# ChengeLi/LongTerm360FoV

Measured on AMD Instinct MI355X. Metric: sequences/sec (batch=1024, T_in=30->T_out=30, h=256), higher is better.
Workload: dtype f32; 1 GPU; configs[1]: target-only seq2seq inference (encoder + autoregressive decoder), H=256, batch=1024 per GPU, T_in=30->T_out=30, F_enc=90, F_dec=6, fp32, act=sigmoid, impl=auto; global_batch=1024, parallelism=replicas x1 (no collective)

## Files before the change

### longterm360fov_amd/csrc/lstm_cluster.hip

```cpp
#include <stdlib.h>

#include <atomic>
#include <mutex>

#include "fov_common.h"
#include "xch_common.h"

namespace fov {

constexpr int BT = 16;
constexpr int XR = 6;
constexpr int KPAD = 2;
constexpr int NXBUF = 3;
constexpr int CL_MAX_F = 96;
constexpr int CL_MAX_O = 8;

constexpr int MODE_LAYER = 0;
constexpr int MODE_DECODE = 1;
constexpr int MODE_LAYER_ZX = 2;

typedef unsigned u32x2 __attribute__((ext_vector_type(2)));
typedef unsigned u32x4g __attribute__((ext_vector_type(4)));
typedef float f32x2 __attribute__((ext_vector_type(2)));
template <bool V> struct BoolC { static constexpr bool value = V; };

__device__ __forceinline__ unsigned long long ld_granule(const unsigned long long* p) {
    return __hip_atomic_load(p, __ATOMIC_RELAXED, __HIP_MEMORY_SCOPE_AGENT);
}
__device__ __forceinline__ void st_granule(unsigned long long* p, unsigned long long v) {
    __hip_atomic_store(p, v, __ATOMIC_RELAXED, __HIP_MEMORY_SCOPE_AGENT);
}
__device__ __forceinline__ void st_granule_l2(unsigned long long* p, unsigned long long v) {
    __hip_atomic_store(p, v, __ATOMIC_RELAXED, __HIP_MEMORY_SCOPE_WORKGROUP);
}
__device__ __forceinline__ unsigned xcc_id() {
    unsigned x;
    asm volatile("s_getreg_b32 %0, hwreg(HW_REG_XCC_ID, 0, 4)" : "=s"(x));
    return x;
}

__host__ __device__ constexpr int round16(int v) { return (v + 15) & ~15; }

#ifdef FOV_STAMPS
constexpr int STAMP_SLOTS = 12;
constexpr int STAMP_STEPS = 64;
__device__ unsigned long long g_stamps[2][STAMP_STEPS][STAMP_SLOTS];
#define FOV_STAMP(slot)                                                                         \
    do {                                                                                        \
        __builtin_amdgcn_sched_barrier(0);                                                      \
        if (stamp_on && t < STAMP_STEPS) {                                                      \
            unsigned long long t_;                                                              \
            asm volatile("s_memtime %0\n\ts_waitcnt lgkmcnt(0)" : "=s"(t_)::"memory");          \
            g_stamps[MODE & 1][t][slot] = t_;                                                       \
        }                                                                                       \
        __builtin_amdgcn_sched_barrier(0);                                                      \
    } while (0)
#define FOV_PSTAMP(slot)                                                                        \
    do {                                                                                        \
        __builtin_amdgcn_sched_barrier(0);                                                      \
        if (blockIdx.x == 5 && threadIdx.x == 0) g_stamps[MODE & 1][STAMP_STEPS - 1][slot] = __builtin_amdgcn_s_memtime(); \
        __builtin_amdgcn_sched_barrier(0);                                                      \
    } while (0)
#else
#define FOV_STAMP(slot) do { } while (0)
#define FOV_PSTAMP(slot) do { } while (0)
#endif

struct ClusterLds {
    int ldx, ldh;
    int off_k, off_h, off_x, off_w, off_bd, off_flag, total_floats;
};
__host__ __device__ inline ClusterLds cluster_lds(int H, int F, bool decode) {
    ClusterLds L;
    const int fp = round16(F);
    L.ldx = fp + 4;
    L.ldh = H + 4;
    L.off_k = 0;
    L.off_h = L.off_k + fp * 256 + 4 * KPAD * 256;
    L.off_x = L.off_h + BT * L.ldh;
    L.off_w = L.off_x + NXBUF * BT * L.ldx;
    L.off_bd = L.off_w + (decode ? 2 * 4 * 128 : 0);
    L.off_flag = L.off_bd + 8;
    L.total_floats = L.off_flag + 8 + 64;
    return L;
}

constexpr int MF_MID = 0, MF_FIRST = 1, MF_LAST = 2;
#define FOV_MFMA_STR(pre, post) pre "v_mfma_f32_16x16x4_f32 %0, %1, %2, %0" post
template <bool W_AGPR>
__device__ __forceinline__ void mfma_f32(f32x4& acc, float a, float w, int pos) {
    if constexpr (W_AGPR) {
        if (pos == MF_MID) asm volatile(FOV_MFMA_STR("", "") : "+v"(acc) : "v"(a), "a"(w));
        else if (pos == MF_FIRST) asm volatile(FOV_MFMA_STR("s_nop 1\n\t", "") : "+v"(acc) : "v"(a), "a"(w));
        else if (pos == MF_LAST) asm volatile(FOV_MFMA_STR("", "\n\ts_nop 7\n\ts_nop 3") : "+v"(acc) : "v"(a), "a"(w));
        else asm volatile(FOV_MFMA_STR("s_nop 1\n\t", "\n\ts_nop 7\n\ts_nop 3") : "+v"(acc) : "v"(a), "a"(w));
    } else {
        if (pos == MF_MID) asm volatile(FOV_MFMA_STR("", "") : "+v"(acc) : "v"(a), "v"(w));
        else if (pos == MF_FIRST) asm volatile(FOV_MFMA_STR("s_nop 1\n\t", "") : "+v"(acc) : "v"(a), "v"(w));
        else if (pos == MF_LAST) asm volatile(FOV_MFMA_STR("", "\n\ts_nop 7\n\ts_nop 3") : "+v"(acc) : "v"(a), "v"(w));
        else asm volatile(FOV_MFMA_STR("s_nop 1\n\t", "\n\ts_nop 7\n\ts_nop 3") : "+v"(acc) : "v"(a), "v"(w));
    }
}
#define FOV_MFMA_C_STR(pre) pre "v_mfma_f32_16x16x4_f32 %0, %1, %2, %3"
template <bool W_AGPR>
__device__ __forceinline__ void mfma_f32_c(f32x4& acc, float a, float w, const f32x4& c, bool a_fresh) {
    if constexpr (W_AGPR) {
        if (a_fresh) asm volatile(FOV_MFMA_C_STR("s_nop 1\n\t") : "=&v"(acc) : "v"(a), "a"(w), "v"(c));
        else asm volatile(FOV_MFMA_C_STR("") : "=&v"(acc) : "v"(a), "a"(w), "v"(c));
    } else {
        if (a_fresh) asm volatile(FOV_MFMA_C_STR("s_nop 1\n\t") : "=&v"(acc) : "v"(a), "v"(w), "v"(c));
        else asm volatile(FOV_MFMA_C_STR("") : "=&v"(acc) : "v"(a), "v"(w), "v"(c));
    }
}
__host__ __device__ constexpr int mf_pos(bool first_run, bool last_run, bool is_first, bool is_last) {
    return ((first_run && is_first) ? MF_FIRST : 0) | ((last_run && is_last) ? MF_LAST : 0);
}

template <int H, bool DEC_KMAP, int J0, int J1, bool REST>
__device__ __forceinline__ void load_weights(float (&wR)[H / 16][4][4], float (&bias)[4], float* sKw,
                                             const float* K, const float* R, const float* b, int F, int Fp,
                                             int col0, int slice, int lane) {
    constexpr int G = H / 64;
    const int n = lane & 15, g4 = lane >> 4;
    const int H4 = 4 * H;
    {
        const __amdgpu_buffer_rsrc_t rrs = __builtin_amdgcn_make_buffer_rsrc(const_cast<float*>(R), 0, H * H4 * 4, 0x00020000);
        const unsigned voff = (unsigned)((4 * g4 * H4 + col0 + n) * 4);
#pragma unroll
        for (int j = J0; j < J1; ++j) {
            const unsigned kb = (unsigned)((((slice + (j >> 2)) & (G - 1)) * 64 + (j & 3) * 16) * H4 * 4);
#pragma unroll
            for (int s = 0; s < 4; ++s)
#pragma unroll
                for (int g = 0; g < 4; ++g)
                    wR[j][s][g] = __uint_as_float(__builtin_amdgcn_raw_buffer_load_b32(rrs, voff, kb + (unsigned)((s * H4 + g * H) * 4), 0));
        }
    }
    if constexpr (!REST) return;
    {
        const __amdgpu_buffer_rsrc_t brs = __builtin_amdgcn_make_buffer_rsrc(const_cast<float*>(b), 0, b ? H4 * 4 : 0, 0x00020000);
#pragma unroll
        for (int g = 0; g < 4; ++g) bias[g] = __uint_as_float(__builtin_amdgcn_raw_buffer_load_b32(brs, (unsigned)((g * H + col0 + n) * 4), 0, 0));
    }
    const int nq = Fp >> 4;
    constexpr int QMAX = CL_MAX_F / 16;
    const __amdgpu_buffer_rsrc_t krs = __builtin_amdgcn_make_buffer_rsrc(const_cast<float*>(K), 0, F * H4 * 4, 0x00020000);
    f32x4 kv[DEC_KMAP ? 1 : QMAX][4];
#pragma unroll
    for (int q = 0; q < (DEC_KMAP ? 1 : QMAX); ++q)
#pragma unroll
        for (int s = 0; s < 4; ++s) {
            const int k = DEC_KMAP ? (s < 2 ? 4 * s + g4 : F) : 16 * q + 4 * g4 + s;
            const unsigned voff = (unsigned)((k * H4 + col0 + n) * 4);
#pragma unroll
            for (int g = 0; g < 4; ++g)
                kv[q][s][g] = __uint_as_float(__builtin_amdgcn_raw_buffer_load_b32(krs, voff + (unsigned)(g * H * 4), 0, 0));
        }
#pragma unroll
    for (int q = 0; q < (DEC_KMAP ? 1 : QMAX); ++q)
        if (q < nq) {
#pragma unroll
            for (int s = 0; s < 4; ++s) *(f32x4*)(sKw + ((q * 4 + s) * 64 + lane) * 4) = kv[q][s];
        }
}

template <int H>
__device__ __forceinline__ void load_r_block(float (&wR)[H / 16][4][4], int j, const float* R, int col0, int slice, int lane) {
    constexpr int G = H / 64;
    const int n = lane & 15, g4 = lane >> 4;
    const int H4 = 4 * H;
    const __amdgpu_buffer_rsrc_t rrs = __builtin_amdgcn_make_buffer_rsrc(const_cast<float*>(R), 0, H * H4 * 4, 0x00020000);
    const unsigned voff = (unsigned)((4 * g4 * H4 + col0 + n) * 4);
    const unsigned kb = (unsigned)((((slice + (j >> 2)) & (G - 1)) * 64 + (j & 3) * 16) * H4 * 4);
#pragma unroll
    for (int s = 0; s < 4; ++s)
#pragma unroll
        for (int g = 0; g < 4; ++g)
            wR[j][s][g] = __uint_as_float(__builtin_amdgcn_raw_buffer_load_b32(rrs, voff, kb + (unsigned)((s * H4 + g * H) * 4), 0));
}
template <int H>
__device__ __forceinline__ void load_dec_small(float (&bias)[4], f32x4 (&kb)[2], const float* K, const float* b, int F, int col0, int lane) {
    const int n = lane & 15, g4 = lane >> 4;
    const int H4 = 4 * H;
    const __amdgpu_buffer_rsrc_t brs = __builtin_amdgcn_make_buffer_rsrc(const_cast<float*>(b), 0, b ? H4 * 4 : 0, 0x00020000);
#pragma unroll
    for (int g = 0; g < 4; ++g) bias[g] = __uint_as_float(__builtin_amdgcn_raw_buffer_load_b32(brs, (unsigned)((g * H + col0 + n) * 4), 0, 0));
    const __amdgpu_buffer_rsrc_t krs = __builtin_amdgcn_make_buffer_rsrc(const_cast<float*>(K), 0, F * H4 * 4, 0x00020000);
#pragma unroll
    for (int s = 0; s < 2; ++s) {
        const unsigned voff = (unsigned)(((4 * s + g4) * H4 + col0 + n) * 4);
#pragma unroll
        for (int g = 0; g < 4; ++g) kb[s][g] = __uint_as_float(__builtin_amdgcn_raw_buffer_load_b32(krs, voff + (unsigned)(g * H * 4), 0, 0));
    }
}

template <bool FIRST, bool LAST, bool CINIT = false>
__device__ __forceinline__ void input_proj(f32x4 (&acc)[4], const float* arow, const float* sKw, int nq, int lane, const f32x4* c0 = nullptr) {
    if (nq <= 0) {
        if constexpr (CINIT) {
#pragma unroll
            for (int g = 0; g < 4; ++g) acc[g] = c0[g];
        }
        return;
    }
    const float* bl = sKw + lane * 4;
    f32x4 a = *(const f32x4*)arow;
    f32x4 b0 = *(const f32x4*)bl;
    f32x4 b1 = *(const f32x4*)(bl + 256);
    if (FIRST && !CINIT) asm volatile("s_nop 1" : "+v"(acc[0]), "+v"(acc[1]), "+v"(acc[2]), "+v"(acc[3]));
    auto block = [&](const int q, auto first_c, auto last_c) __attribute__((always_inline)) {
        constexpr bool C0 = decltype(first_c)::value, LB = decltype(last_c)::value;
        const float* bq = bl + q * 1024;
#pragma unroll
        for (int s = 0; s < 4; ++s) {
            const f32x4 bn = *(const f32x4*)(bq + (s + 2) * 256);
#pragma unroll
            for (int g = 0; g < 4; ++g) {
                if (C0 && s == 0) mfma_f32_c<false>(acc[g], a[s], b0[g], c0[g], false);
                else mfma_f32<false>(acc[g], a[s], b0[g], mf_pos(false, LB && LAST, false, s == 3 && g == 3));
            }
            b0 = b1;
            b1 = bn;
        }
    };
    int q = 0;
    if constexpr (CINIT) {
        const f32x4 an = *(const f32x4*)(arow + 16);
        block(0, BoolC<true>{}, BoolC<true>{});
        if (nq == 1) return;
        a = an;
        q = 1;
    }
    for (; q < nq - 1; ++q) {
        const f32x4 an = *(const f32x4*)(arow + 16 * (q + 1));
        block(q, BoolC<false>{}, BoolC<false>{});
        a = an;
    }
    block(nq - 1, BoolC<false>{}, BoolC<true>{});
}

template <int NQC, bool FIRST, bool LAST, bool CINIT = false>
__device__ __forceinline__ void input_proj_fixed(f32x4 (&acc)[4], const float* arow, const float* sKw, int lane, const f32x4* c0 = nullptr) {
    const float* bl = sKw + lane * 4;
    f32x4 a = *(const f32x4*)arow;
    f32x4 b0 = *(const f32x4*)bl;
    f32x4 b1 = *(const f32x4*)(bl + 256);
#pragma unroll
    for (int q = 0; q < NQC; ++q) {
        f32x4 an = a;
        if (q + 1 < NQC) an = *(const f32x4*)(arow + 16 * (q + 1));
#pragma unroll
        for (int s = 0; s < 4; ++s) {
            f32x4 bn = b1;
            if (4 * q + s + 2 < 4 * NQC) bn = *(const f32x4*)(bl + (4 * q + s + 2) * 256);
#pragma unroll
            for (int g = 0; g < 4; ++g) {
                if (CINIT && q == 0 && s == 0) mfma_f32_c<false>(acc[g], a[s], b0[g], c0[g], false);
                else mfma_f32<false>(acc[g], a[s], b0[g], mf_pos(FIRST && !CINIT, LAST, q == 0 && s == 0, q == NQC - 1 && s == 3 && g == 3));
            }
            b0 = b1;
            b1 = bn;
        }
        a = an;
    }
}
template <bool FIRST, bool LAST, bool CINIT = false>
__device__ __forceinline__ void input_proj_any(f32x4 (&acc)[4], const float* arow, const float* sKw, int nq, int lane, const f32x4* c0 = nullptr) {
    if (nq == 6) input_proj_fixed<6, FIRST, LAST, CINIT>(acc, arow, sKw, lane, c0);
    else input_proj<FIRST, LAST, CINIT>(acc, arow, sKw, nq, lane, c0);
}

template <bool LAST, bool CINIT = false>
__device__ __forceinline__ void input_proj_reg(f32x4 (&acc)[4], f32x4 y4, const f32x4 (&kb)[2], const f32x4* c0 = nullptr) {
#pragma unroll
    for (int s = 0; s < 2; ++s)
#pragma unroll
        for (int g = 0; g < 4; ++g) {
            if (CINIT && s == 0) mfma_f32_c<false>(acc[g], y4[s], kb[s][g], c0[g], true);
            else mfma_f32<false>(acc[g], y4[s], kb[s][g], mf_pos(true, LAST, s == 0, s == 1 && g == 3));
        }
}

template <int H, int J0, int J1, bool FIRST, bool LAST, bool CINIT = false>
__device__ __forceinline__ void recurrent(f32x4 (&acc)[4], const float* hrow, const float (&wR)[H / 16][4][4], const f32x4* c0 = nullptr) {
    if (J0 >= J1) return;
    f32x4 a = *(const f32x4*)(hrow + 16 * J0);
#pragma unroll
    for (int j = J0; j < J1; ++j) {
        f32x4 an = a;
        if (j + 1 < J1) an = *(const f32x4*)(hrow + 16 * (j + 1));
#pragma unroll
        for (int s = 0; s < 4; ++s)
#pragma unroll
            for (int g = 0; g < 4; ++g) {
                if (CINIT && j == J0 && s == 0) mfma_f32_c<true>(acc[g], a[s], wR[j][s][g], c0[g], false);
                else mfma_f32<true>(acc[g], a[s], wR[j][s][g], mf_pos(FIRST && !CINIT, LAST, j == J0 && s == 0, j == J1 - 1 && s == 3 && g == 3));
            }
        a = an;
    }
}

struct ClusterCarry {
    unsigned epoch;
    XchTicket ticket;
    bool same_xcd, aborted, xch_used;
    float c[4], h[4];
};

template <int H, int ACT, int MODE, int FUSED>
__device__ __forceinline__ void cluster_body(const LstmParams& p, ClusterCarry& cy) {
    constexpr int G = H / 64;
    constexpr int NQ = H / 16;
    constexpr int NG = (G - 1) * 2;
    constexpr bool LAYER = (MODE != MODE_DECODE);
    constexpr bool ZX = (MODE == MODE_LAYER_ZX);
    constexpr bool F1 = (FUSED == 1), F2 = (FUSED == 2);
    constexpr bool FZ = (FUSED != 0);
    extern __shared__ __attribute__((aligned(16))) float smem[];

    const int tid = threadIdx.x, lane = tid & 63, wave = tid >> 6;
    const int n = lane & 15, g4 = lane >> 4;
    constexpr unsigned OORB = 0x80000000u;
#ifdef FOV_STAMPS
    if (blockIdx.x == 5 && tid == 0) g_stamps[MODE & 1][STAMP_STEPS - 1][0] = __builtin_amdgcn_s_memtime();
#endif
    float hcarry[BT * H / 256];
    if constexpr (F2) {
        const ClusterLds L1 = cluster_lds(H, p.F, false);
#pragma unroll
        for (int q = 0; q < BT * H / 256; ++q) {
            const int i = tid + 256 * q;
            hcarry[q] = smem[L1.off_h + (i / H) * L1.ldh + (i - (i / H) * H)];
        }
        __syncthreads();
    }
    int group, slice;
    if (G > 1 && ((p.num_groups & 7) == 0 || p.xcd_pad)) {
        group = (blockIdx.x / (8 * G)) * 8 + (blockIdx.x & 7);
        slice = (blockIdx.x >> 3) & (G - 1);
    } else {
        group = blockIdx.x / G;
        slice = blockIdx.x - group * G;
    }
    const int col0 = slice * 64 + wave * 16;

    const float* Kp = LAYER ? p.K : p.dK;
    const float* Rp = LAYER ? p.R : p.dR;
    const float* bp = LAYER ? p.b : p.db;
    const int F = LAYER ? (ZX ? 0 : p.F) : p.F_dec;
    const int steps = LAYER ? p.T : p.T_out;
    const int Fp = round16(F);
    const int nq = Fp >> 4;

    const ClusterLds L = cluster_lds(H, F, !LAYER);
    const int LDX = L.ldx, LDH = L.ldh;
    float* sK = smem + L.off_k;
    float* sH = smem + L.off_h;
    float* sX = smem + L.off_x;
    float* sY = smem + L.off_w;
    int* sFlag = (int*)(smem + L.off_flag);
    float* sKw = sK + wave * (nq * 4 + KPAD) * 256;

    const bool xch_used = (G > 1) && (!LAYER || p.T > 1 || F1);
    unsigned* sXch = (unsigned*)(sFlag + 4);
    const bool hdr = xch_used && !F2;
    unsigned hdr_base = 0, hdr_launch = 0;
    if (hdr && tid == 0) {
        hdr_base = xch_status_load(p.status + ST_EPOCH);
        hdr_launch = xch_status_load(p.status + ST_LAUNCHES);
    }
    float wR[NQ][4][4];
    float bias[4];
    constexpr int JA = NQ < 3 ? NQ : 3;
    constexpr int STREAM_LA = 3;
    f32x4 kb[2];
    if constexpr (F2) {
        load_dec_small<H>(bias, kb, Kp, bp, F, col0, lane);
    } else {
        load_weights<H, !LAYER, 0, JA, false>(wR, bias, sKw, Kp, Rp, bp, F, Fp, col0, slice, lane);
    }
    unsigned long long* hello = p.xch + (size_t)p.num_groups * 2 * BT * H + (size_t)group * G;
    const unsigned my_xcc = xcc_id();
    if (hdr && tid == 0) {
        sXch[0] = hdr_base;
        sXch[1] = hdr_launch;
        st_granule(hello + slice, (((unsigned long long)hdr_base + 1ull) << 32) | my_xcc);
        xch_count_arrival(p.status);
    }
    FOV_PSTAMP(3);
    if constexpr (!F2) load_weights<H, !LAYER, JA, NQ, true>(wR, bias, sKw, Kp, Rp, bp, F, Fp, col0, slice, lane);
    FOV_PSTAMP(2);
    const bool poisoned = hdr && xch_poisoned(p.status);
    if (tid == 0) { sFlag[0] = (poisoned || (F2 && cy.aborted)) ? 1 : 0; sFlag[1] = 0; }
    if (hdr && !poisoned && tid < G) {
        const unsigned long long hello_tag = (unsigned long long)sXch[0] + 1ull;
        unsigned long long hv = 0;
        unsigned spins = 0;
        while (true) {
            hv = ld_granule(hello + tid);
            if ((hv >> 32) == hello_tag) break;
            if (xch_wait_expired(++spins, p.status)) {
                xch_give_up(p.status);
                sFlag[0] = 1;
                break;
            }
            __builtin_amdgcn_s_sleep(4);
        }
        if ((unsigned)hv != my_xcc) sFlag[1] = 1;
    }
    FOV_PSTAMP(4);
    float xpre[2][XR];
    {
        const int xrw0 = tid >> 4, xcl0 = tid & 15;
        const bool xuse0 = LAYER && !ZX;
        const int b00 = group * BT;
        const int live0 = (group < p.num_tiles) ? (p.B - b00 < BT ? p.B - b00 : BT) : 0;
        const __amdgpu_buffer_rsrc_t xg0 = __builtin_amdgcn_make_buffer_rsrc(
            const_cast<float*>(xuse0 && live0 > 0 ? p.x + (size_t)b00 * p.T * F : nullptr), 0, xuse0 ? live0 * p.T * F * 4 : 0, 0x00020000);
#pragma unroll
        for (int tt = 0; tt < 2; ++tt)
#pragma unroll
            for (int i = 0; i < XR; ++i)
                xpre[tt][i] = __uint_as_float(__builtin_amdgcn_raw_buffer_load_b32(
                    xg0, (tt < steps && xcl0 + 16 * i < F) ? (unsigned)((xrw0 * p.T * F + xcl0 + 16 * i) * 4) : OORB, (unsigned)(tt * F * 4), 0));
    }
    for (int i = tid; i < NXBUF * BT * LDX; i += 256) sX[i] = 0.f;

    float wd[4];
    float bd4[4];
    if (!LAYER) {
        const int O = p.F_dec;
        const __amdgpu_buffer_rsrc_t wdrs = __builtin_amdgcn_make_buffer_rsrc(const_cast<float*>(p.dW), 0, H * O * 4, 0x00020000);
        const __amdgpu_buffer_rsrc_t bdrs = __builtin_amdgcn_make_buffer_rsrc(const_cast<float*>(p.dbias), 0, O * 4, 0x00020000);
#pragma unroll
        for (int ss = 0; ss < 4; ++ss) {
            const int unit = col0 + 4 * g4 + ss;
            const int o = 4 * (n & 3) + (n >> 2);
            wd[ss] = __uint_as_float(__builtin_amdgcn_raw_buffer_load_b32(wdrs, (o < O) ? (unsigned)((unit * O + o) * 4) : OORB, 0, 0));
        }
#pragma unroll
        for (int ss = 0; ss < 4; ++ss)
            bd4[ss] = __uint_as_float(__builtin_amdgcn_raw_buffer_load_b32(bdrs, (4 * ss + g4 < O) ? (unsigned)((4 * ss + g4) * 4) : OORB, 0, 0));
    }
    if constexpr (F2) {
#pragma unroll
        for (int j = 0; j < STREAM_LA; ++j) load_r_block<H>(wR, j, Rp, col0, slice, lane);
    } else if (!LAYER) {
        __syncthreads();
        kb[0] = *(const f32x4*)(sKw + lane * 4);
        kb[1] = *(const f32x4*)(sKw + 256 + lane * 4);
    }

    __syncthreads();
    FOV_PSTAMP(5);
    XchTicket ticket = {0u, 0u, false};
    if (xch_used && !F2) ticket = xch_ticket(sXch);
    if constexpr (F2) ticket = cy.ticket;
    unsigned epoch = F2 ? cy.epoch : ticket.base;
    const bool same_xcd = F2 ? cy.same_xcd : (xch_used && (sFlag[1] == 0) && (p.force_safe_exchange == 0));
    bool aborted = F2 ? cy.aborted : (xch_used && sFlag[0] != 0);
    if (xch_used && !F2 && tid == 0 && !same_xcd && !aborted)
        xch_count_safe(p.status, ticket);
#ifdef FOV_STAMPS
    const bool stamp_on = (blockIdx.x == 5 && tid == 0);
#endif
    const float* hrow = sH + n * LDH + 4 * g4;

    const __amdgpu_buffer_rsrc_t xrs = __builtin_amdgcn_make_buffer_rsrc(
        p.xch + (size_t)group * 2 * BT * H, 0, 2 * BT * H * (int)sizeof(unsigned long long), 0x00020000);
    const unsigned pub_off = (unsigned)((2 * g4) * H + col0 + n) * 16u;
    unsigned goff[NG > 0 ? NG : 1];
    int loff[NG > 0 ? NG : 1];
#pragma unroll
    for (int j = 0; j < NG; ++j) {
        const int idx = j * 256 + tid;
        const int rot = (idx >> 9) + 1, within = idx & 511;
        const int osl = (slice + rot) & (G - 1);
        goff[j] = (unsigned)((within >> 6) * H + osl * 64 + (within & 63)) * 16u;
        loff[j] = 2 * (within >> 6) * LDH + rot * 64 + (within & 63);
    }

    constexpr int NYG = (LAYER || G == 1) ? 0 : G;
    const __amdgpu_buffer_rsrc_t yrs = __builtin_amdgcn_make_buffer_rsrc(
        p.xch + (size_t)p.num_groups * 2 * BT * H + (size_t)p.num_groups * G + (size_t)group * 2 * G * 128, 0,
        LAYER ? 0 : 2 * G * 128 * (int)sizeof(unsigned long long), 0x00020000);
    const unsigned ypub_off = (unsigned)((slice * 64 + lane) * 16);
    const unsigned ygoff = (unsigned)(lane * 16);
    constexpr unsigned YPAR_BYTES = G * 64 * 16;
    constexpr int YPAR_LDS = 4 * 128;
    auto own_partial = [&](int par) -> f32x2 {
        const float* yb = sY + par * YPAR_LDS + lane * 2;
        const f32x2 a0 = *(const f32x2*)yb, a1 = *(const f32x2*)(yb + 128), a2 = *(const f32x2*)(yb + 256), a3 = *(const f32x2*)(yb + 384);
        return (a0 + a1) + (a2 + a3);
    };

    const bool h_zero = F1 || (!F2 && p.h0 == nullptr);
    for (int tile = group; tile < p.num_tiles && !aborted; tile += p.num_groups) {
        const int b0 = tile * BT;
        const int live_rows = p.B - b0 < BT ? p.B - b0 : BT;
        const __amdgpu_buffer_rsrc_t c0rs = __builtin_amdgcn_make_buffer_rsrc(
            const_cast<float*>(p.c0 ? p.c0 + (size_t)b0 * H : nullptr), 0, p.c0 ? live_rows * H * 4 : 0, 0x00020000);
        const __amdgpu_buffer_rsrc_t h0rs = __builtin_amdgcn_make_buffer_rsrc(
            const_cast<float*>(p.h0 ? p.h0 + (size_t)b0 * H : nullptr), 0, p.h0 ? live_rows * H * 4 : 0, 0x00020000);
        float c[4], hcur[4];
#pragma unroll
        for (int r = 0; r < 4; ++r) {
            const unsigned off = (unsigned)(((4 * g4 + r) * H + col0 + n) * 4);
            if constexpr (F2) {
                c[r] = cy.c[r];
                hcur[r] = cy.h[r];
            } else {
                c[r] = __uint_as_float(__builtin_amdgcn_raw_buffer_load_b32(c0rs, off, 0, 0));
                hcur[r] = __uint_as_float(__builtin_amdgcn_raw_buffer_load_b32(h0rs, off, 0, 0));
            }
        }
        {
            float hv[BT * H / 256];
#pragma unroll
            for (int q = 0; q < BT * H / 256; ++q) {
                const int i = tid + 256 * q;
                const int row = i / H, pos = i - row * H;
                const int unit = ((slice + (pos >> 6)) & (G - 1)) * 64 + (pos & 63);
                if constexpr (F2) hv[q] = hcarry[q];
                else hv[q] = h_zero ? 0.f : __uint_as_float(__builtin_amdgcn_raw_buffer_load_b32(h0rs, (unsigned)((row * H + unit) * 4), 0, 0));
            }
#pragma unroll
            for (int q = 0; q < BT * H / 256; ++q) {
                const int i = tid + 256 * q;
                const int row = i / H, pos = i - row * H;
                sH[row * LDH + pos] = hv[q];
            }
        }
        const int xrw = tid >> 4, xcl = tid & 15;
        const bool xuse = LAYER && !ZX;
        const __amdgpu_buffer_rsrc_t xgrs = __builtin_amdgcn_make_buffer_rsrc(
            const_cast<float*>(xuse ? p.x + (size_t)b0 * p.T * F : nullptr), 0, xuse ? live_rows * p.T * F * 4 : 0, 0x00020000);
        unsigned xoff[XR];
#pragma unroll
        for (int i = 0; i < XR; ++i) xoff[i] = (xcl + 16 * i < F) ? (unsigned)((xrw * p.T * F + xcl + 16 * i) * 4) : OORB;
        const __amdgpu_buffer_rsrc_t zxrs = __builtin_amdgcn_make_buffer_rsrc(
            const_cast<float*>(ZX ? p.zx + (size_t)b0 * p.T * 4 * H : nullptr), 0, ZX ? live_rows * p.T * 4 * H * 4 : 0, 0x00020000);
        const unsigned zxoff = (unsigned)((4 * g4 * p.T * 4 * H + col0 + n) * 4);
        f32x4 zr[4];
        float* xl = sX + xrw * LDX + xcl;
        if (xuse) {
            float x2[2][XR];
            if (tile == group) {
#pragma unroll
                for (int tt = 0; tt < 2; ++tt)
#pragma unroll
                    for (int i = 0; i < XR; ++i) x2[tt][i] = xpre[tt][i];
            } else {
#pragma unroll
                for (int tt = 0; tt < 2; ++tt)
#pragma unroll
                    for (int i = 0; i < XR; ++i)
                        x2[tt][i] = __uint_as_float(__builtin_amdgcn_raw_buffer_load_b32(xgrs, tt < steps ? xoff[i] : OORB, (unsigned)(tt * F * 4), 0));
            }
#pragma unroll
            for (int tt = 0; tt < 2; ++tt)
                if (tt < steps) {
#pragma unroll
                    for (int i = 0; i < XR; ++i)
                        if (xcl + 16 * i < F) xl[tt * BT * LDX + 16 * i] = x2[tt][i];
                }
        }
        const __amdgpu_buffer_rsrc_t yors = __builtin_amdgcn_make_buffer_rsrc(
            (!LAYER && p.out) ? p.out + (size_t)b0 * p.T_out * p.F_dec : nullptr, 0, (!LAYER && p.out) ? live_rows * p.T_out * p.F_dec * 4 : 0, 0x00020000);
        unsigned yoff[2];
#pragma unroll
        for (int ss = 0; ss < 2; ++ss)
            yoff[ss] = (!LAYER && 4 * ss + g4 < p.F_dec && (!F2 || (slice == 0 && wave == 0))) ? (unsigned)((n * p.T_out * p.F_dec + 4 * ss + g4) * 4) : OORB;
        f32x4 y4 = (f32x4){0.f, 0.f, 0.f, 0.f};
        if (!LAYER) {
            const __amdgpu_buffer_rsrc_t y0rs = __builtin_amdgcn_make_buffer_rsrc(
                const_cast<float*>(p.dec_in0 + (size_t)b0 * F), 0, live_rows * F * 4, 0x00020000);
#pragma unroll
            for (int ss = 0; ss < 4; ++ss)
                y4[ss] = __uint_as_float(__builtin_amdgcn_raw_buffer_load_b32(y0rs, (4 * ss + g4 < F) ? (unsigned)((n * F + 4 * ss + g4) * 4) : OORB, 0, 0));
        }
        __syncthreads();
        FOV_PSTAMP(6);

        f32x4 bias4[4];
#pragma unroll
        for (int g = 0; g < 4; ++g) bias4[g] = (f32x4){bias[g], bias[g], bias[g], bias[g]};
        asm volatile("" : "+v"(bias4[0]), "+v"(bias4[1]), "+v"(bias4[2]), "+v"(bias4[3]));
        f32x4 acc[4];
#pragma unroll
        for (int g = 0; g < 4; ++g) acc[g] = bias4[g];
        if (ZX && steps > 0) {
#pragma unroll
            for (int g = 0; g < 4; ++g)
#pragma unroll
                for (int r = 0; r < 4; ++r)
                    acc[g][r] = bias[g] + __uint_as_float(__builtin_amdgcn_raw_buffer_load_b32(zxrs, zxoff + (unsigned)((r * p.T * 4 * H + g * H) * 4), 0, 0));
        }
        if (steps > 0) {
            if constexpr (ZX) input_proj_any<true, true>(acc, sX + n * LDX + 4 * g4, sKw, nq, lane);
            else if constexpr (LAYER) input_proj_any<true, true, true>(acc, sX + n * LDX + 4 * g4, sKw, nq, lane, bias4);
            else input_proj_reg<true, true>(acc, y4, kb, bias4);
            if constexpr (F2) {
                f32x4 a = *(const f32x4*)hrow;
#pragma unroll
                for (int j = 0; j < NQ; ++j) {
                    if (j + STREAM_LA < NQ) load_r_block<H>(wR, j + STREAM_LA, Rp, col0, slice, lane);
                    f32x4 an = a;
                    if (j + 1 < NQ) an = *(const f32x4*)(hrow + 16 * (j + 1));
#pragma unroll
                    for (int s2 = 0; s2 < 4; ++s2)
#pragma unroll
                        for (int g = 0; g < 4; ++g)
                            mfma_f32<true>(acc[g], a[s2], wR[j][s2][g], mf_pos(false, true, false, j == NQ - 1 && s2 == 3 && g == 3));
                    a = an;
                }
            } else if (!h_zero) {
                recurrent<H, 0, 4, true, true>(acc, hrow, wR);
            }
        }

        float xr[XR];
#pragma unroll
        for (int i = 0; i < XR; ++i) xr[i] = 0.f;
        auto step = [&](const int t, auto st_c) __attribute__((always_inline)) -> bool {
            constexpr bool ST = decltype(st_c)::value;
            const bool t_pos = ST || t > 0;
            const bool more = ST || (t + 1 < steps);
            const bool more2 = ST || (t + 2 < steps);
            const bool sxcd = ST || same_xcd;
            FOV_STAMP(0);
#ifdef FOV_STAMPS
            if (stamp_on && t < STAMP_STEPS) g_stamps[MODE & 1][t][9] = __builtin_amdgcn_s_memrealtime();
#endif
            if (LAYER && !ZX && t_pos && more) {
                float* xb = xl + ((t + 1) % 3) * BT * LDX;
#pragma unroll
                for (int i = 0; i < XR; ++i)
                    if (ST || xcl + 16 * i < F) xb[16 * i] = xr[i];
            }
            if (ZX && more) {
#pragma unroll
                for (int g = 0; g < 4; ++g)
#pragma unroll
                    for (int r = 0; r < 4; ++r)
                        zr[g][r] = bias[g] + __uint_as_float(__builtin_amdgcn_raw_buffer_load_b32(
                                                 zxrs, zxoff + (unsigned)(((r * p.T + (t + 1)) * 4 * H + g * H) * 4), 0, 0));
            }
            if (LAYER && !ZX && more2) {
#pragma unroll
                for (int i = 0; i < XR; ++i)
                    xr[i] = __uint_as_float(__builtin_amdgcn_raw_buffer_load_b32(xgrs, xoff[i], (unsigned)((t + 2) * F * 4), 0));
            }
            if (LAYER || (!ST && t == 0)) {
                if (ST || !((h_zero || F2) && t == 0)) recurrent<H, 4, NQ, true, true>(acc, hrow, wR);
            } else {
                constexpr int JM = 4 + (NQ - 4) / 2;
                recurrent<H, 4, JM, true, false>(acc, hrow, wR);
                u32x4g vy[NYG > 0 ? NYG : 1];
                const unsigned yso = (epoch & 1u) * YPAR_BYTES;
#pragma unroll
                for (int q = 0; q < NYG; ++q) vy[q] = __builtin_amdgcn_raw_buffer_load_b128(yrs, ygoff, yso + (unsigned)(q * 1024), 16);
                recurrent<H, JM, NQ, false, false>(acc, hrow, wR);
                __builtin_amdgcn_sched_barrier(0);
                f32x2 ysum;
                if constexpr (NYG > 0) {
                    unsigned spins = 0;
                    auto ytags_ok = [&]() __attribute__((always_inline)) -> bool {
                        bool ok = true;
#pragma unroll
                        for (int q = 0; q < NYG; ++q) ok = ok && (vy[q].y == epoch) && (vy[q].w == epoch);
                        return __all(ok);
                    };
                    if (!ytags_ok()) {
                        while (true) {
                            if (xch_wait_expired(++spins, p.status)) {
                                if (lane == 0) { xch_give_up(p.status); sFlag[0] = 1; }
                                break;
                            }
                            __builtin_amdgcn_s_sleep(1);
                            asm volatile("" ::: "memory");
#pragma unroll
                            for (int q = 0; q < NYG; ++q) vy[q] = __builtin_amdgcn_raw_buffer_load_b128(yrs, ygoff, yso + (unsigned)(q * 1024), 16);
                            asm volatile("");
                            if (ytags_ok()) break;
                        }
                    }
                    f32x2 P[NYG];
#pragma unroll
                    for (int q = 0; q < NYG; ++q) P[q] = (f32x2){__uint_as_float(vy[q].x), __uint_as_float(vy[q].z)};
#pragma unroll
                    for (int w2 = NYG / 2; w2 >= 1; w2 >>= 1)
#pragma unroll
                        for (int q = 0; q < w2; ++q) P[q] += P[q + w2];
                    ysum = P[0];
                } else {
                    ysum = own_partial((t - 1) & 1);
                }
#pragma unroll
                for (int ss = 0; ss < 2; ++ss) y4[ss] = tanh_f(ysum[ss] + bd4[ss]);
                if (ST || (slice == 0 && wave == 0)) {
#pragma unroll
                    for (int ss = 0; ss < 2; ++ss)
                        __builtin_amdgcn_raw_buffer_store_b32(__float_as_uint(y4[ss]), yors, yoff[ss], (unsigned)((t - 1) * p.F_dec * 4), 0);
                }
                __builtin_amdgcn_sched_barrier(0);
                input_proj_reg<true>(acc, y4, kb);
            }
            FOV_STAMP(1);
#pragma unroll
            for (int r = 0; r < 4; ++r) {
#ifdef FOV_DBG_NOCELL
                const float ig = acc[0][r], fg = acc[1][r], gg = acc[2][r], og = acc[3][r];
                c[r] = fmaf(fg, c[r], ig * gg);
                hcur[r] = og * c[r];
#else
                const float ig = rec_act<ACT>(acc[0][r]);
                const float fg = rec_act<ACT>(acc[1][r]);
                const float gg = tanh_f(acc[2][r]);
                const float og = rec_act<ACT>(acc[3][r]);
                c[r] = fmaf(fg, c[r], ig * gg);
                hcur[r] = og * tanh_f(c[r]);
#endif
                if (LAYER && !FZ && p.reserve) {
                    const int row = b0 + 4 * g4 + r;
                    if (row < p.B) {
                        float* rp = p.reserve + (((size_t)row * p.T + t) * 5) * H + col0 + n;
                        rp[0] = ig; rp[H] = fg; rp[2 * H] = gg; rp[3 * H] = og; rp[4 * H] = c[r];
                    }
                }
            }
            unsigned xsoff = 0;
            const bool do_xch = (G > 1) && (!LAYER || more || F1);
            if (do_xch) {
                ++epoch;
                xsoff = (epoch & 1u) * (unsigned)(BT * H * sizeof(unsigned long long));
                if (sxcd) {
#pragma unroll
                    for (int r = 0; r < 2; ++r)
                        __builtin_amdgcn_raw_buffer_store_b128((u32x4g){__float_as_uint(hcur[2 * r]), epoch, __float_as_uint(hcur[2 * r + 1]), epoch},
                                                               xrs, pub_off + r * H * 16, xsoff, 1 );
                } else {
#pragma unroll
                    for (int r = 0; r < 2; ++r)
                        __builtin_amdgcn_raw_buffer_store_b128((u32x4g){__float_as_uint(hcur[2 * r]), epoch, __float_as_uint(hcur[2 * r + 1]), epoch},
                                                               xrs, pub_off + r * H * 16, xsoff, 16 );
                }
            }
            if (LAYER && !FZ && p.hs) {
#pragma unroll
                for (int r = 0; r < 4; ++r) {
                    const int row = b0 + 4 * g4 + r;
                    if (row < p.B) p.hs[((size_t)row * p.T + t) * H + col0 + n] = hcur[r];
                }
            }
            FOV_STAMP(2);
            FOV_STAMP(3);
#pragma unroll
            for (int r = 0; r < 4; ++r) sH[(4 * g4 + r) * LDH + wave * 16 + n] = hcur[r];
            __syncthreads();
            FOV_STAMP(4);
            if (more) {
                const float* xa = sX + ((t + 1) % 3) * BT * LDX + n * LDX + 4 * g4;
                if constexpr (ZX) {
#pragma unroll
                    for (int g = 0; g < 4; ++g) acc[g] = zr[g];
                } else if constexpr (LAYER && ST) {
                    input_proj_fixed<6, true, false, true>(acc, xa, sKw, lane, bias4);
                } else if constexpr (LAYER) {
// ... 137 lines not shown
                if (got) {
#pragma unroll
                    for (int ss = 0; ss < 2; ++ss)
                        __builtin_amdgcn_raw_buffer_store_b32(__float_as_uint(tanh_f(ysum[ss] + bd4[ss])), yors, yoff[ss],
                                                              (unsigned)((steps - 1) * p.F_dec * 4), 0);
                }
            }
        }
        if constexpr (F1) {
#pragma unroll
            for (int r = 0; r < 4; ++r) { cy.c[r] = c[r]; cy.h[r] = hcur[r]; }
        }
        if (!aborted && !F1) {
#pragma unroll
            for (int r = 0; r < 4; ++r) {
                const int row = b0 + 4 * g4 + r;
                if (row < p.B) {
                    if (p.hT) p.hT[(size_t)row * H + col0 + n] = hcur[r];
                    if (p.cT) p.cT[(size_t)row * H + col0 + n] = c[r];
                }
            }
        }
#ifdef FOV_STAMPS
        if (blockIdx.x == 5 && tid == 0) g_stamps[MODE & 1][STAMP_STEPS - 1][1] = __builtin_amdgcn_s_memtime();
#endif
        if constexpr (FUSED != 0) break;
    }
    if constexpr (F1) {
        cy.epoch = epoch; cy.ticket = ticket; cy.same_xcd = same_xcd; cy.aborted = aborted; cy.xch_used = xch_used;
        __syncthreads();
    } else {
        if (xch_used) xch_settle(p.status, ticket, (unsigned)p.epoch_span);
    }
}

template <int H, int ACT, int MODE>
__global__ __launch_bounds__(256, 1) void lstm_cluster_kernel(LstmParams p) {
    if constexpr (H >= 128) {
        if (p.xcd_pad && (int)((blockIdx.x / (8 * (H / 64))) * 8 + (blockIdx.x & 7)) >= p.num_groups) {
            const bool exchanging = (MODE == MODE_DECODE) || p.T > 1;
            if (threadIdx.x == 0 && exchanging) xch_count_arrival(p.status);
            return;
        }
    }
    ClusterCarry cy;
    cluster_body<H, ACT, MODE, 0>(p, cy);
}

template <int H, int ACT>
__global__ __launch_bounds__(256, 1) void lstm_cluster_fused_kernel(LstmParams p) {
    if constexpr (H >= 128) {
        if (p.xcd_pad && (int)((blockIdx.x / (8 * (H / 64))) * 8 + (blockIdx.x & 7)) >= p.num_groups) {
            if (threadIdx.x == 0) xch_count_arrival(p.status);
            return;
        }
    }
    ClusterCarry cy;
    cluster_body<H, ACT, MODE_LAYER, 1>(p, cy);
    cluster_body<H, ACT, MODE_DECODE, 2>(p, cy);
}

int device_cu_count() {
    static std::atomic<int> cus[64];
    int dev = 0, n = 256;
    if (hipGetDevice(&dev) == hipSuccess && dev >= 0 && dev < 64 && (n = cus[dev].load(std::memory_order_relaxed)) == 0) {
        hipDeviceProp_t prop;
        n = (hipGetDeviceProperties(&prop, dev) == hipSuccess && prop.multiProcessorCount > 0) ? prop.multiProcessorCount : 256;
        cus[dev].store(n, std::memory_order_relaxed);
    }
    const int lim = env_knobs().resident_limit;
    return (lim > 0 && lim < n) ? lim : n;
}

int ensure_dynamic_lds(const void* kern, size_t lds, int block) {
    struct Seen { const void* k; size_t lds; int dev; };
    static Seen seen[256];
    static int n_seen = 0;
    static std::mutex mu;
    int dev = 0;
    (void)hipGetDevice(&dev);
    std::lock_guard<std::mutex> lock(mu);
    for (int i = 0; i < n_seen; ++i)
        if (seen[i].k == kern && seen[i].dev == dev && seen[i].lds >= lds) return FOV_OK;
    hipError_t e = hipFuncSetAttribute(kern, hipFuncAttributeMaxDynamicSharedMemorySize, (int)lds);
    if (e != hipSuccess) { set_error("hipFuncSetAttribute: %s", hipGetErrorString(e)); return FOV_ERR_LAUNCH; }
    int per_cu = 0;
    e = hipOccupancyMaxActiveBlocksPerMultiprocessor(&per_cu, kern, block, lds);
    if (e != hipSuccess || per_cu < 1) {
        (void)hipGetLastError();
        set_error("persistent kernel: a %d-thread workgroup with %zu B of LDS is not resident on this device (occupancy %d)", block, lds, per_cu);
        return FOV_ERR_UNSUPPORTED;
    }
    if (n_seen < 256) seen[n_seen++] = Seen{kern, lds, dev};
    return FOV_OK;
}

bool cluster_shape_ok(int F, int H) {
    return (H == 64 || H == 128 || H == 256) && F >= 1 && F <= CL_MAX_F;
}

int cluster_num_groups(int B, int H) {
    const int G = H / 64;
    const int tiles = (B + BT - 1) / BT;
    const int groups = device_cu_count() / G;
    if (groups < 1) return 0;
    return tiles < groups ? (tiles > 0 ? tiles : 1) : groups;
}

static size_t cluster_xch_bytes(int B, int H) {
    const size_t groups = (size_t)cluster_num_groups(B, H);
    const size_t b = (groups * 2 * BT * H + groups * (H / 64) + groups * 2 * (H / 64) * 128) * sizeof(unsigned long long);
    return (b + 255) & ~(size_t)255;
}

size_t cluster_workspace_bytes(int B, int H) {
    (void)cluster_xch_bytes;
    return kStatusBytes + kXchBytes + (size_t)2 * B * H * sizeof(float);
}

template <int H>
static int launch_cluster_h(const LstmParams& p, int mode, hipStream_t stream) {
    void (*kern)(LstmParams) = nullptr;
    if (mode == MODE_LAYER && p.zx) mode = MODE_LAYER_ZX;
    if (p.act == FOV_ACT_HARD_SIGMOID)
        kern = mode == MODE_DECODE ? lstm_cluster_kernel<H, FOV_ACT_HARD_SIGMOID, MODE_DECODE>
               : mode == MODE_LAYER_ZX ? lstm_cluster_kernel<H, FOV_ACT_HARD_SIGMOID, MODE_LAYER_ZX>
                                       : lstm_cluster_kernel<H, FOV_ACT_HARD_SIGMOID, MODE_LAYER>;
    else
        kern = mode == MODE_DECODE ? lstm_cluster_kernel<H, FOV_ACT_SIGMOID, MODE_DECODE>
               : mode == MODE_LAYER_ZX ? lstm_cluster_kernel<H, FOV_ACT_SIGMOID, MODE_LAYER_ZX>
                                       : lstm_cluster_kernel<H, FOV_ACT_SIGMOID, MODE_LAYER>;
    const int F = mode == MODE_DECODE ? p.F_dec : (p.zx ? 0 : p.F);
    const ClusterLds L = cluster_lds(H, F, mode == MODE_DECODE);
    const size_t lds = (size_t)L.total_floats * sizeof(float);
    if (lds > 160 * 1024) {
        set_error("cluster kernel: H=%d F=%d needs %zu B of LDS (> 160 KiB)", H, F, lds);
        return FOV_ERR_UNSUPPORTED;
    }
    int rc = ensure_dynamic_lds((const void*)kern, lds);
    if (rc) return rc;
    LstmParams q = p;
    const int padded = xch_padded_groups(q.num_groups);
    q.xcd_pad = (H >= 128 && !env_knobs().no_xcd_pad && (q.num_groups & 7) != 0 && device_cu_count() >= padded * (H / 64)) ? 1 : 0;
    const dim3 grid((q.xcd_pad ? padded : q.num_groups) * (H / 64)), block(256);
    hipLaunchKernelGGL(kern, grid, block, lds, stream, q);
    return launch_check("cluster");
}

template <int H>
static int launch_cluster_fused_h(const LstmParams& p, hipStream_t stream) {
    void (*kern)(LstmParams) = p.act == FOV_ACT_HARD_SIGMOID ? lstm_cluster_fused_kernel<H, FOV_ACT_HARD_SIGMOID>
                                                             : lstm_cluster_fused_kernel<H, FOV_ACT_SIGMOID>;
    const ClusterLds L1 = cluster_lds(H, p.F, false), L2 = cluster_lds(H, p.F_dec, true);
    const size_t lds = (size_t)(L1.total_floats > L2.total_floats ? L1.total_floats : L2.total_floats) * sizeof(float);
    if (lds > 160 * 1024) { set_error("fused cluster kernel: needs %zu B of LDS (> 160 KiB)", lds); return FOV_ERR_UNSUPPORTED; }
    int rc = ensure_dynamic_lds((const void*)kern, lds);
    if (rc) return rc;
    LstmParams q = p;
    const bool no_pad = env_knobs().no_xcd_pad != 0;
    const int padded = (q.num_groups + 7) & ~7;
    q.xcd_pad = (H >= 128 && !no_pad && (q.num_groups & 7) != 0 && device_cu_count() >= padded * (H / 64)) ? 1 : 0;
    hipLaunchKernelGGL(kern, dim3((q.xcd_pad ? padded : q.num_groups) * (H / 64)), dim3(256), lds, stream, q);
    return launch_check("fused cluster");
}

static int launch_cluster_fused(const LstmParams& p, hipStream_t stream) {
    switch (p.H) {
        case 64: return launch_cluster_fused_h<64>(p, stream);
        case 128: return launch_cluster_fused_h<128>(p, stream);
        default: return launch_cluster_fused_h<256>(p, stream);
    }
}

static int launch_cluster_mode(const LstmParams& p, int mode, hipStream_t stream) {
    switch (p.H) {
        case 64: return launch_cluster_h<64>(p, mode, stream);
        case 128: return launch_cluster_h<128>(p, mode, stream);
        default: return launch_cluster_h<256>(p, mode, stream);
    }
}

int launch_cluster(const LstmParams& p_in, bool decode, hipStream_t stream) {
    LstmParams p = p_in;
    if (p.B == 0) return FOV_OK;
    if (p.zx) p.F = 1;
    if (!cluster_shape_ok(p.F, p.H) || (decode && (p.F_dec < 1 || p.F_dec > CL_MAX_O))) {
        set_error("cluster kernel supports H in {64,128,256}, 1<=F<=%d, F_dec<=%d (got H=%d F=%d F_dec=%d)",
                  CL_MAX_F, CL_MAX_O, p.H, p.F, p.F_dec);
        return FOV_ERR_UNSUPPORTED;
    }
    p.num_tiles = (p.B + BT - 1) / BT;
    p.num_groups = cluster_num_groups(p.B, p.H);
    if (p.num_groups < 1) { set_error("cluster kernel: fewer than %d CUs available for one group", p.H / 64); return FOV_ERR_UNSUPPORTED; }
    p.force_safe_exchange = env_knobs().force_safe_exchange;
    if (cluster_xch_bytes(p.B, p.H) > kXchBytes - kHelloBytes) { set_error("cluster kernel: granule area exceeds the workspace's"); return FOV_ERR_WORKSPACE; }
    const int visits = (p.num_tiles + p.num_groups - 1) / p.num_groups;
    if (!decode) {
        p.epoch_span = p.T * visits + 1;
        if (int rc_ = xch_account(p.status, p.epoch_span, stream)) return rc_;
        return launch_cluster_mode(p, MODE_LAYER, stream);
    }

    if (visits == 1 && p.T > 0 && p.T_out > 0 && !p.hs && !p.reserve && !p.h0 && !env_knobs().two_launches) {
        LstmParams f = p;
        f.epoch_span = p.T + p.T_out + 2;
        if (int rc_ = xch_account(p.status, f.epoch_span, stream)) return rc_;
        return launch_cluster_fused(f, stream);
    }
    LstmParams enc = p;
    float* state = (float*)((char*)p.status + kStatusBytes + kXchBytes);
    enc.hT = state;
    enc.cT = state + (size_t)p.B * p.H;
    enc.hs = nullptr;
    enc.epoch_span = p.T * visits + 1;
    if (int rc_ = xch_account(p.status, enc.epoch_span + p.T_out * visits + 1, stream)) return rc_;
    int rc = launch_cluster_mode(enc, MODE_LAYER, stream);
    if (rc) return rc;
    LstmParams dec = p;
    dec.h0 = enc.hT;
    dec.c0 = enc.cT;
    dec.epoch_span = p.T_out * visits + 1;
    return launch_cluster_mode(dec, MODE_DECODE, stream);
}

int launch_cluster_decoder(const LstmParams& p_in, hipStream_t stream) {
    LstmParams p = p_in;
    if (p.B == 0 || p.T_out == 0) return FOV_OK;
    if (!(p.H == 64 || p.H == 128 || p.H == 256) || p.F_dec < 1 || p.F_dec > CL_MAX_O) {
        set_error("cluster decoder supports H in {64,128,256}, F_dec<=%d (got H=%d F_dec=%d)", CL_MAX_O, p.H, p.F_dec);
        return FOV_ERR_UNSUPPORTED;
    }
    p.num_tiles = (p.B + BT - 1) / BT;
    p.num_groups = cluster_num_groups(p.B, p.H);
    if (p.num_groups < 1) { set_error("cluster decoder: fewer than %d CUs available for one group", p.H / 64); return FOV_ERR_UNSUPPORTED; }
    p.force_safe_exchange = env_knobs().force_safe_exchange;
    p.epoch_span = p.T_out * ((p.num_tiles + p.num_groups - 1) / p.num_groups) + 1;
    if (int rc_ = xch_account(p.status, p.epoch_span, stream)) return rc_;
    return launch_cluster_mode(p, MODE_DECODE, stream);
}

#ifdef FOV_STAMPS
extern "C" int fov_debug_read_stamps(unsigned long long* out) {
    return (int)hipMemcpyFromSymbol(out, HIP_SYMBOL(g_stamps), sizeof(unsigned long long) * 2 * STAMP_STEPS * STAMP_SLOTS);
}
#endif

}
```

Measured before the change: 3.165 million sequences/s.

## Stage cluster LSTM weights via coalesced b128 loads through an LDS ring

Replaces the per-lane scalar b32 gathers of recurrent and input weights with wide b128 buffer loads, kept up to seven stages deep in flight. Each R block is transposed through a swizzled, double-buffered LDS ring into the MFMA register layout, and K is written directly to LDS with a rotated layout. In the fused decoder phase the LDS stores are interleaved with the first recurrent MFMA blocks so the weight load overlaps compute. This adds LDS use and a barrier per block in exchange for fewer memory transactions during weight loading.

```diff
diff --git a/longterm360fov_amd/csrc/lstm_cluster.hip b/longterm360fov_amd/csrc/lstm_cluster.hip
--- a/longterm360fov_amd/csrc/lstm_cluster.hip
+++ b/longterm360fov_amd/csrc/lstm_cluster.hip
@@ -14,6 +14,10 @@
 constexpr int NXBUF = 3;
 constexpr int CL_MAX_F = 96;
 constexpr int CL_MAX_O = 8;
+constexpr int WST_WORDS = 20;
+constexpr int WST_BUF = 256 * WST_WORDS;
+constexpr int WST_RING = 2 * WST_BUF;
+constexpr int WST_DEPTH = 7;
 
 constexpr int MODE_LAYER = 0;
 constexpr int MODE_DECODE = 1;
@@ -80,7 +84,7 @@
     L.off_x = L.off_h + BT * L.ldh;
     L.off_w = L.off_x + NXBUF * BT * L.ldx;
     L.off_bd = L.off_w + (decode ? 2 * 4 * 128 : 0);
-    L.off_flag = L.off_bd + 8;
+    L.off_flag = L.off_bd + 8 > L.off_h + WST_RING ? L.off_bd + 8 : L.off_h + WST_RING;
     L.total_floats = L.off_flag + 8 + 64;
     return L;
 }
@@ -116,75 +120,102 @@
     return ((first_run && is_first) ? MF_FIRST : 0) | ((last_run && is_last) ? MF_LAST : 0);
 }
 
-template <int H, bool DEC_KMAP, int J0, int J1, bool REST>
-__device__ __forceinline__ void load_weights(float (&wR)[H / 16][4][4], float (&bias)[4], float* sKw,
-                                             const float* K, const float* R, const float* b, int F, int Fp,
-                                             int col0, int slice, int lane) {
-    constexpr int G = H / 64;
-    const int n = lane & 15, g4 = lane >> 4;
-    const int H4 = 4 * H;
-    {
-        const __amdgpu_buffer_rsrc_t rrs = __builtin_amdgcn_make_buffer_rsrc(const_cast<float*>(R), 0, H * H4 * 4, 0x00020000);
-        const unsigned voff = (unsigned)((4 * g4 * H4 + col0 + n) * 4);
-#pragma unroll
-        for (int j = J0; j < J1; ++j) {
-            const unsigned kb = (unsigned)((((slice + (j >> 2)) & (G - 1)) * 64 + (j & 3) * 16) * H4 * 4);
-#pragma unroll
-            for (int s = 0; s < 4; ++s)
-#pragma unroll
-                for (int g = 0; g < 4; ++g)
-                    wR[j][s][g] = __uint_as_float(__builtin_amdgcn_raw_buffer_load_b32(rrs, voff, kb + (unsigned)((s * H4 + g * H) * 4), 0));
-        }
-    }
-    if constexpr (!REST) return;
-    {
-        const __amdgpu_buffer_rsrc_t brs = __builtin_amdgcn_make_buffer_rsrc(const_cast<float*>(b), 0, b ? H4 * 4 : 0, 0x00020000);
-#pragma unroll
-        for (int g = 0; g < 4; ++g) bias[g] = __uint_as_float(__builtin_amdgcn_raw_buffer_load_b32(brs, (unsigned)((g * H + col0 + n) * 4), 0, 0));
-    }
-    const int nq = Fp >> 4;
-    constexpr int QMAX = CL_MAX_F / 16;
-    const __amdgpu_buffer_rsrc_t krs = __builtin_amdgcn_make_buffer_rsrc(const_cast<float*>(K), 0, F * H4 * 4, 0x00020000);
-    f32x4 kv[DEC_KMAP ? 1 : QMAX][4];
-#pragma unroll
-    for (int q = 0; q < (DEC_KMAP ? 1 : QMAX); ++q)
-#pragma unroll
-        for (int s = 0; s < 4; ++s) {
-            const int k = DEC_KMAP ? (s < 2 ? 4 * s + g4 : F) : 16 * q + 4 * g4 + s;
-            const unsigned voff = (unsigned)((k * H4 + col0 + n) * 4);
-#pragma unroll
-            for (int g = 0; g < 4; ++g)
-                kv[q][s][g] = __uint_as_float(__builtin_amdgcn_raw_buffer_load_b32(krs, voff + (unsigned)(g * H * 4), 0, 0));
-        }
-#pragma unroll
-    for (int q = 0; q < (DEC_KMAP ? 1 : QMAX); ++q)
-        if (q < nq) {
-#pragma unroll
-            for (int s = 0; s < 4; ++s) *(f32x4*)(sKw + ((q * 4 + s) * 64 + lane) * 4) = kv[q][s];
-        }
+struct WstAllStores {
+    template <class Store>
+    __device__ __forceinline__ void operator()(int, Store store) const {
+#pragma unroll
+        for (int k = 0; k < 16; ++k) store(k);
+    }
+};
+typedef unsigned wst_u32x4 __attribute__((ext_vector_type(4)));
+template <int H, bool HAS_K, class Behind, class Under>
+__device__ __forceinline__ void stage_cluster_weights(float (&wR)[H / 16][4][4], const float* R, const float* K, int F, int nq,
+                                                      float* sK, unsigned* ring, int slice, Behind behind_first_loads,
+                                                      Under under_stores) {
+    constexpr int G = H / 64, NQ = H / 16, QK = HAS_K ? CL_MAX_F / 16 : 0, NS = QK + NQ;
+    constexpr int DEPTH = WST_DEPTH < NS ? WST_DEPTH : NS;
+    constexpr unsigned ROWB = 4 * H * 4;
+    const int tid = threadIdx.x, lane = tid & 63, wave = tid >> 6, n = lane & 15, g4 = lane >> 4;
+    const int c = (lane & 7) + 8 * (lane >> 5), kr = (lane >> 3) & 3;
+    const __amdgpu_buffer_rsrc_t rrs = __builtin_amdgcn_make_buffer_rsrc(const_cast<float*>(R), 0, H * ROWB, 0x00020000);
+    const __amdgpu_buffer_rsrc_t krs = __builtin_amdgcn_make_buffer_rsrc(const_cast<float*>(K), 0, HAS_K ? F * ROWB : 0, 0x00020000);
+    const unsigned goff = (unsigned)(kr * 4 * H + wave * H + 64 * slice + 4 * c) * 4u;
+    const int fw = ((c ^ (c >> 1)) & 1) | (((c >> 2) & 1) << 1);
+    unsigned wofs[4];
+#pragma unroll
+    for (int it = 0; it < 4; ++it) wofs[it] = (unsigned)((64 * wave + 4 * c) * WST_WORDS + kr + 4 * (it ^ fw));
+    const int fr = (((n >> 2) ^ (n >> 3)) & 1) | ((wave & 1) << 1);
+    const unsigned rofs = (unsigned)((16 * wave + n) * WST_WORDS + 4 * (g4 ^ fr));
+    const int kgate = (lane >> 3) & 3, krot = (c >> 1) & 3;
+    const unsigned kgoff = (unsigned)(wave * 4 * H + kgate * H + 64 * slice + 4 * c) * 4u;
+    float* kdst = sK + (c >> 2) * (nq * 4 + KPAD) * 256 + wave * 256 + 16 * (c & 3) + kgate;
+    int kx[4];
+#pragma unroll
+    for (int t = 0; t < 4; ++t) kx[t] = 4 * (t ^ krot);
+
+    wst_u32x4 r[DEPTH + 1][4];
+    auto issue = [&](const int s) __attribute__((always_inline)) {
+        if (s < QK) {
+#pragma unroll
+            for (int it = 0; it < 4; ++it)
+                r[s % (DEPTH + 1)][it] = __builtin_amdgcn_raw_buffer_load_b128(krs, kgoff + (unsigned)(16 * s + 4 * it) * ROWB, 0, 0);
+        } else {
+            const int j = s - QK;
+            const unsigned k0 = (unsigned)((((slice + (j >> 2)) & (G - 1)) * 64 + (j & 3) * 16)) * ROWB;
+#pragma unroll
+            for (int it = 0; it < 4; ++it)
+                r[s % (DEPTH + 1)][it] = __builtin_amdgcn_raw_buffer_load_b128(rrs, goff + k0 + (unsigned)(4 * it) * ROWB, 0, 0);
+        }
+    };
+#pragma unroll
+    for (int s = 0; s < DEPTH; ++s) {
+        issue(s);
+        if (s == (DEPTH < 3 ? DEPTH : 3) - 1) behind_first_loads();
+    }
+#pragma unroll
+    for (int s = 0; s < NS; ++s) {
+        if (s + DEPTH < NS) issue(s + DEPTH);
+        const wst_u32x4(&v)[4] = r[s % (DEPTH + 1)];
+        if (s < QK) {
+            if (s < nq) {
+#pragma unroll
+                for (int it = 0; it < 4; ++it) {
+                    const bool r0 = krot & 1, r1 = krot & 2;
+                    const unsigned a0 = r0 ? v[it][1] : v[it][0], a1 = r0 ? v[it][0] : v[it][1];
+                    const unsigned a2 = r0 ? v[it][3] : v[it][2], a3 = r0 ? v[it][2] : v[it][3];
+                    const unsigned u[4] = {r1 ? a2 : a0, r1 ? a3 : a1, r1 ? a0 : a2, r1 ? a1 : a3};
+#pragma unroll
+                    for (int t = 0; t < 4; ++t) kdst[s * 1024 + it * 64 + kx[t]] = __uint_as_float(u[t]);
+                }
+            }
+        } else {
+            const int j = s - QK;
+            unsigned* buf = ring + (j & 1) * WST_BUF;
+            under_stores(j, [&](const int k) __attribute__((always_inline)) { buf[wofs[k >> 2] + (k & 3) * WST_WORDS] = v[k >> 2][k & 3]; });
+            __syncthreads();
+#pragma unroll
+            for (int g = 0; g < 4; ++g) {
+                const wst_u32x4 w4 = *(const wst_u32x4*)(buf + rofs + g * 64 * WST_WORDS);
+#pragma unroll
+                for (int sub = 0; sub < 4; ++sub) wR[j][sub][g] = __uint_as_float(w4[sub]);
+            }
+        }
+    }
+    __syncthreads();
 }
 
 template <int H>
-__device__ __forceinline__ void load_r_block(float (&wR)[H / 16][4][4], int j, const float* R, int col0, int slice, int lane) {
-    constexpr int G = H / 64;
-    const int n = lane & 15, g4 = lane >> 4;
-    const int H4 = 4 * H;
-    const __amdgpu_buffer_rsrc_t rrs = __builtin_amdgcn_make_buffer_rsrc(const_cast<float*>(R), 0, H * H4 * 4, 0x00020000);
-    const unsigned voff = (unsigned)((4 * g4 * H4 + col0 + n) * 4);
-    const unsigned kb = (unsigned)((((slice + (j >> 2)) & (G - 1)) * 64 + (j & 3) * 16) * H4 * 4);
-#pragma unroll
-    for (int s = 0; s < 4; ++s)
-#pragma unroll
-        for (int g = 0; g < 4; ++g)
-            wR[j][s][g] = __uint_as_float(__builtin_amdgcn_raw_buffer_load_b32(rrs, voff, kb + (unsigned)((s * H4 + g * H) * 4), 0));
+__device__ __forceinline__ void load_bias(float (&bias)[4], const float* b, int col0, int lane) {
+    const int n = lane & 15;
+    const __amdgpu_buffer_rsrc_t brs = __builtin_amdgcn_make_buffer_rsrc(const_cast<float*>(b), 0, b ? 4 * H * 4 : 0, 0x00020000);
+#pragma unroll
+    for (int g = 0; g < 4; ++g) bias[g] = __uint_as_float(__builtin_amdgcn_raw_buffer_load_b32(brs, (unsigned)((g * H + col0 + n) * 4), 0, 0));
 }
 template <int H>
 __device__ __forceinline__ void load_dec_small(float (&bias)[4], f32x4 (&kb)[2], const float* K, const float* b, int F, int col0, int lane) {
     const int n = lane & 15, g4 = lane >> 4;
     const int H4 = 4 * H;
-    const __amdgpu_buffer_rsrc_t brs = __builtin_amdgcn_make_buffer_rsrc(const_cast<float*>(b), 0, b ? H4 * 4 : 0, 0x00020000);
-#pragma unroll
-    for (int g = 0; g < 4; ++g) bias[g] = __uint_as_float(__builtin_amdgcn_raw_buffer_load_b32(brs, (unsigned)((g * H + col0 + n) * 4), 0, 0));
+    load_bias<H>(bias, b, col0, lane);
     const __amdgpu_buffer_rsrc_t krs = __builtin_amdgcn_make_buffer_rsrc(const_cast<float*>(K), 0, F * H4 * 4, 0x00020000);
 #pragma unroll
     for (int s = 0; s < 2; ++s) {
@@ -371,24 +402,24 @@
     }
     float wR[NQ][4][4];
     float bias[4];
-    constexpr int JA = NQ < 3 ? NQ : 3;
-    constexpr int STREAM_LA = 3;
     f32x4 kb[2];
-    if constexpr (F2) {
-        load_dec_small<H>(bias, kb, Kp, bp, F, col0, lane);
-    } else {
-        load_weights<H, !LAYER, 0, JA, false>(wR, bias, sKw, Kp, Rp, bp, F, Fp, col0, slice, lane);
-    }
+    if constexpr (LAYER) load_bias<H>(bias, bp, col0, lane);
+    else load_dec_small<H>(bias, kb, Kp, bp, F, col0, lane);
     unsigned long long* hello = p.xch + (size_t)p.num_groups * 2 * BT * H + (size_t)group * G;
     const unsigned my_xcc = xcc_id();
-    if (hdr && tid == 0) {
-        sXch[0] = hdr_base;
-        sXch[1] = hdr_launch;
-        st_granule(hello + slice, (((unsigned long long)hdr_base + 1ull) << 32) | my_xcc);
-        xch_count_arrival(p.status);
-    }
-    FOV_PSTAMP(3);
-    if constexpr (!F2) load_weights<H, !LAYER, JA, NQ, true>(wR, bias, sKw, Kp, Rp, bp, F, Fp, col0, slice, lane);
+    if constexpr (!F2) {
+        stage_cluster_weights<H, LAYER && !ZX>(wR, Rp, Kp, F, nq, sK, (unsigned*)sH, slice, [&]() __attribute__((always_inline)) {
+            if (hdr && tid == 0) {
+                sXch[0] = hdr_base;
+                sXch[1] = hdr_launch;
+                st_granule(hello + slice, (((unsigned long long)hdr_base + 1ull) << 32) | my_xcc);
+                xch_count_arrival(p.status);
+            }
+            FOV_PSTAMP(3);
+        }, WstAllStores{});
+    } else {
+        FOV_PSTAMP(3);
+    }
     FOV_PSTAMP(2);
     const bool poisoned = hdr && xch_poisoned(p.status);
     if (tid == 0) { sFlag[0] = (poisoned || (F2 && cy.aborted)) ? 1 : 0; sFlag[1] = 0; }
@@ -442,14 +473,6 @@
         for (int ss = 0; ss < 4; ++ss)
             bd4[ss] = __uint_as_float(__builtin_amdgcn_raw_buffer_load_b32(bdrs, (4 * ss + g4 < O) ? (unsigned)((4 * ss + g4) * 4) : OORB, 0, 0));
     }
-    if constexpr (F2) {
-#pragma unroll
-        for (int j = 0; j < STREAM_LA; ++j) load_r_block<H>(wR, j, Rp, col0, slice, lane);
-    } else if (!LAYER) {
-        __syncthreads();
-        kb[0] = *(const f32x4*)(sKw + lane * 4);
-        kb[1] = *(const f32x4*)(sKw + 256 + lane * 4);
-    }
 
     __syncthreads();
     FOV_PSTAMP(5);
@@ -602,18 +625,25 @@
             else input_proj_reg<true, true>(acc, y4, kb, bias4);
             if constexpr (F2) {
                 f32x4 a = *(const f32x4*)hrow;
-#pragma unroll
-                for (int j = 0; j < NQ; ++j) {
-                    if (j + STREAM_LA < NQ) load_r_block<H>(wR, j + STREAM_LA, Rp, col0, slice, lane);
+                auto block = [&](const int j, auto store) __attribute__((always_inline)) {
                     f32x4 an = a;
                     if (j + 1 < NQ) an = *(const f32x4*)(hrow + 16 * (j + 1));
 #pragma unroll
                     for (int s2 = 0; s2 < 4; ++s2)
 #pragma unroll
-                        for (int g = 0; g < 4; ++g)
+                        for (int g = 0; g < 4; ++g) {
                             mfma_f32<true>(acc[g], a[s2], wR[j][s2][g], mf_pos(false, true, false, j == NQ - 1 && s2 == 3 && g == 3));
+                            store(4 * s2 + g);
+                        }
                     a = an;
-                }
+                };
+                stage_cluster_weights<H, false>(wR, Rp, Kp, F, nq, sK, (unsigned*)(smem + L.total_floats), slice, []() {},
+                                                [&](const int j, auto store) __attribute__((always_inline)) {
+                                                    if (j >= 2) block(j - 2, store);
+                                                    else WstAllStores{}(j, store);
+                                                });
+                block(NQ - 2, [](int) {});
+                block(NQ - 1, [](int) {});
             } else if (!h_zero) {
                 recurrent<H, 0, 4, true, true>(acc, hrow, wR);
             }
@@ -1057,7 +1087,8 @@
     void (*kern)(LstmParams) = p.act == FOV_ACT_HARD_SIGMOID ? lstm_cluster_fused_kernel<H, FOV_ACT_HARD_SIGMOID>
                                                              : lstm_cluster_fused_kernel<H, FOV_ACT_SIGMOID>;
     const ClusterLds L1 = cluster_lds(H, p.F, false), L2 = cluster_lds(H, p.F_dec, true);
-    const size_t lds = (size_t)(L1.total_floats > L2.total_floats ? L1.total_floats : L2.total_floats) * sizeof(float);
+    const int dec_floats = L2.total_floats + WST_RING;
+    const size_t lds = (size_t)(L1.total_floats > dec_floats ? L1.total_floats : dec_floats) * sizeof(float);
     if (lds > 160 * 1024) { set_error("fused cluster kernel: needs %zu B of LDS (> 160 KiB)", lds); return FOV_ERR_UNSUPPORTED; }
     int rc = ensure_dynamic_lds((const void*)kern, lds);
     if (rc) return rc;
```

New measurement: 3.185 million sequences/s (median of 6 runs). No clear change (+0.6%).
